# lipku/LiveTalking

Hardware: NVIDIA H100
Metric: lip-sync frames/sec (wav2lip256, 256x256, batch 16, mel + U-Net fwd + paste-back) (higher is better)
Workload: dtype f16 (fp32 accumulate); mel f64; paste u8

## Files before the change

### include/ltb200.h

```cpp
#ifndef LTB200_H_
#define LTB200_H_

#include <stddef.h>
#include <stdint.h>

#ifdef __cplusplus
extern "C" {
#endif

typedef struct ltb_w2l_model ltb_w2l_model;
typedef struct ltb_w2l_avatar ltb_w2l_avatar;
typedef struct ltb_w2l_session ltb_w2l_session;

int ltb_version(void);
const char* ltb_last_error(void);
int ltb_device_count(int* count);
int ltb_set_device(int device);

int ltb_w2l_model_create(const void* blob, size_t nbytes, ltb_w2l_model** out);
int ltb_w2l_model_create_from_device(void* blob_dev, size_t nbytes, ltb_w2l_model** out);
int ltb_w2l_model_destroy(ltb_w2l_model* m);

int ltb_w2l_avatar_create(const uint8_t* faces, const uint8_t* frames, const int32_t* coords, int n, int H, int W,
                          ltb_w2l_avatar** out);
// ... 57 lines not shown
int ltb_ctx_destroy(ltb_ctx* c);
int ltb_ctx_stream(ltb_ctx* c, void** cuda_stream);
int ltb_ctx_sync(ltb_ctx* c);
int ltb_ctx_launch_count(ltb_ctx* c, long long* n);
int ltb_dev_alloc(ltb_ctx* c, size_t bytes, int zero, void** dptr);
int ltb_dev_free(ltb_ctx* c, void* dptr);
int ltb_h2d(ltb_ctx* c, void* dst_dev, const void* src_host, size_t bytes, int sync);
int ltb_d2h(ltb_ctx* c, void* dst_host, const void* src_dev, size_t bytes, int sync);
int ltb_set_i32(ltb_ctx* c, void* dptr, int value);
int ltb_capture_begin(ltb_ctx* c);
int ltb_capture_end(ltb_ctx* c, ltb_graph** out);
int ltb_graph_launch(ltb_ctx* c, ltb_graph* g);
int ltb_graph_destroy(ltb_graph* g);

int ltb_d2d(ltb_ctx* c, void* dst_dev, const void* src_dev, size_t bytes);
typedef struct ltb_conv_op {
  const void* in; const void* w; const void* w_tap; const float* bias; const void* res; void* out;
  int N, IH, IW, ICtot, ic_off, Cin;
  int OH, OW, Cout, OCtot, oc_off, RCtot, rc_off;
  int KH, KW, sy, sx, pad_t, pad_l;
  int Ktot, w_koff, relu, no_halo;
  int zbatch, zdiv;
  long long in_zo, in_zi, w_zo, w_zi, out_zo, out_zi;
  void* gn_stats;
  int gn_groups, gn_hw;
  int upsample2x;
  const int* group_slot;
  int group_images, slots;
  long long w_slot_stride, bias_slot_stride;
  int transposed;
} ltb_conv_op;
int ltb_op_conv2d(ltb_ctx* c, const ltb_conv_op* d);
typedef struct ltb_conv_variant {
  int kernel, taps, bn, nsub, nacc, resident_chunks, kb, ksplit, grouped, res_halo;
} ltb_conv_variant;
int ltb_op_conv2d_plan(ltb_ctx* c, const ltb_conv_op* d, ltb_conv_variant* out);
int ltb_op_w_tap_major(ltb_ctx* c, const void* w, void* wt, int cout, int cin);
int ltb_op_groupnorm(ltb_ctx* c, const void* x, int N, int HW, int C, int Ctot, int c_off, int groups, float eps, const float* gamma,
                     const float* beta, int silu, void* out, int OCtot, int oc_off);
int ltb_op_groupnorm_apply(ltb_ctx* c, const void* x, int N, int HW, int C, int Ctot, int c_off, int groups, float eps, const void* stats,
                           const float* gamma, const float* beta, int silu, void* out, int OCtot, int oc_off);
int ltb_op_layernorm(ltb_ctx* c, const void* x, int rows, int C, float eps, const float* gamma, const float* beta, void* out);
int ltb_op_softmax(ltb_ctx* c, const void* x, int rows, int cols, int ld, int valid, float scale, void* out);
int ltb_op_geglu(ltb_ctx* c, const void* h, long long rows, int H, void* out);
int ltb_op_eltwise(ltb_ctx* c, const void* x, const void* y, long long n, long long period, int act, void* out);
int ltb_op_upsample2x(ltb_ctx* c, const void* x, int N, int H, int W, int C, void* out);
int ltb_op_copy_channels(ltb_ctx* c, const void* src, long long rows, int C, int SCtot, int sc_off, void* dst, int DCtot, int dc_off);
int ltb_op_transpose_heads(ltb_ctx* c, const void* v, int B, int n_keys, int Ctot, int c_off, int heads, int d, int n_pad, void* vt);
int ltb_op_attention(ltb_ctx* c, const void* q, int q_pitch, const void* k, int kv_pitch, int kv_rows, const void* vt, int n_pad, int B, int heads,
                     int nq, int valid, int d, float scale, void* out, int out_pitch);
int ltb_op_dwconv3x3(ltb_ctx* c, const void* x, int N, int IH, int IW, int ICtot, int ic_off, int C, const void* w_tap, const float* bias, int stride,
                     int relu, void* out, int OCtot, int oc_off);
int ltb_op_dwconv3x3_grouped(ltb_ctx* c, const void* x, int N, int IH, int IW, int ICtot, int ic_off, int C, const void* w_tap, const float* bias,
                             int stride, int relu, void* out, int OCtot, int oc_off, const int* group_slot, int group_images, long long w_slot_stride,
                             long long bias_slot_stride);
int ltb_op_upsample_bilinear2x(ltb_ctx* c, const void* x, int N, int H, int W, int ICtot, int ic_off, int C, void* out, int OCtot, int oc_off);
int ltb_op_ul_prep(ltb_ctx* c, const void* faces_u8, int nf, const void* d_index, int B, void* out);
typedef struct ltb_ul_prep_group {
  const void* faces;
  int nf, index;
} ltb_ul_prep_group;
int ltb_op_ul_prep_grouped(ltb_ctx* c, const void* groups_dev, int group_images, int B, void* out);
int ltb_op_head_sigmoid255(ltb_ctx* c, const void* x, const float* w3x32, const float* b3, long long npix, float* pred);
int ltb_op_head_sigmoid255_grouped(ltb_ctx* c, const void* x, const float* w3x32, const float* b3, long long npix, float* pred, int hw,
                                   const int* group_slot, int group_images, long long w_slot_stride, long long bias_slot_stride);
int ltb_op_ul_paste(ltb_ctx* c, const void* frames, const void* faces, const void* coords, const float* pred, void* out, int nf, int H, int W,
                    int index, int explicit_idx, int slot0, int count);
// ... 38 lines not shown
```

### livetalking_b200/_capi.py

```python
from __future__ import annotations

import ctypes as C
import os

_HERE = os.path.dirname(os.path.abspath(__file__))
LIB_PATH = os.path.join(_HERE, "lib", "libltb200.so")

LTB_SESSION_KEEP_LAYERS = 1
LTB_SESSION_NO_GRAPH = 2
LTB_SESSION_NO_HALO = 4
LTB_SESSION_NO_PDL = 8
LTB_SESSION_SLOTS = 16
LTB_SESSION_MEL_ONLY = 32


class LtbError(RuntimeError):
    pass


class ConvOp(C.Structure):
    _fields_ = ([(n, C.c_void_p) for n in ("in_", "w", "w_tap", "bias", "res", "out")] +
                [(n, C.c_int) for n in ("N", "IH", "IW", "ICtot", "ic_off", "Cin", "OH", "OW", "Cout", "OCtot", "oc_off", "RCtot",
                                        "rc_off", "KH", "KW", "sy", "sx", "pad_t", "pad_l", "Ktot", "w_koff", "relu", "no_halo",
                                        "zbatch", "zdiv")] +
                [(n, C.c_longlong) for n in ("in_zo", "in_zi", "w_zo", "w_zi", "out_zo", "out_zi")] +
                [("gn_stats", C.c_void_p), ("gn_groups", C.c_int), ("gn_hw", C.c_int), ("upsample2x", C.c_int)] +
                [("group_slot", C.c_void_p), ("group_images", C.c_int), ("slots", C.c_int), ("w_slot_stride", C.c_longlong),
                 ("bias_slot_stride", C.c_longlong), ("transposed", C.c_int)])


class ConvVariant(C.Structure):
    _fields_ = [(n, C.c_int) for n in ("kernel", "taps", "bn", "nsub", "nacc", "resident_chunks", "kb", "ksplit", "grouped", "res_halo")]


class UlPrepGroup(C.Structure):
    _fields_ = [("faces", C.c_void_p), ("nf", C.c_int), ("index", C.c_int)]


class MtPasteOp(C.Structure):
    _fields_ = ([(n, C.c_void_p) for n in ("frames", "coords", "crop", "masks", "mask_off", "pred", "out")] +
                [(n, C.c_int) for n in ("nf", "H", "W", "index", "explicit_idx", "slot0", "count", "pred_hw")])


class W2LSlot(C.Structure):
    _fields_ = [("avatar", C.c_void_p), ("idx", C.c_int), ("mel", C.c_void_p)]


class ConvDesc(C.Structure):
    _fields_ = [(n, C.c_int) for n in
                ("N", "IH", "IW", "Cin", "Cout", "KH", "KW", "sy", "sx", "pad", "transposed", "relu", "has_res",
                 "force_path")]


_SIGS = {
    "ltb_version": (C.c_int, []),
    "ltb_last_error": (C.c_char_p, []),
    "ltb_device_count": (C.c_int, [C.POINTER(C.c_int)]),
    "ltb_set_device": (C.c_int, [C.c_int]),
    "ltb_w2l_model_create": (C.c_int, [C.c_void_p, C.c_size_t, C.POINTER(C.c_void_p)]),
    "ltb_w2l_model_create_from_device": (C.c_int, [C.c_void_p, C.c_size_t, C.POINTER(C.c_void_p)]),
    "ltb_w2l_model_destroy": (C.c_int, [C.c_void_p]),
    "ltb_w2l_avatar_create": (C.c_int, [C.c_void_p, C.c_void_p, C.c_void_p, C.c_int, C.c_int, C.c_int,
                                        C.POINTER(C.c_void_p)]),
    "ltb_w2l_avatar_destroy": (C.c_int, [C.c_void_p]),
    "ltb_w2l_session_create": (C.c_int, [C.c_void_p, C.c_void_p, C.c_int, C.c_int, C.c_int, C.c_int, C.c_int,
# ... 128 lines not shown
```

### livetalking_b200/csrc/conv_gather.cu

```cuda
#include "conv_params.h"
#include "ltb_internal.h"
#include "ptx_sm90.cuh"

namespace ltb {

constexpr int kGatherThreads = 256;

template <int BN, int KB>
struct GatherCfg {
  static constexpr int CH = KB / 8;
  static constexpr int ROWB = KB * 2;
  static constexpr int RSTEP = kGatherThreads / CH;
  static constexpr int RPT = 128 / RSTEP;
  static constexpr int A_BYTES = 128 * ROWB;
  static constexpr int B_BYTES = (BN * ROWB < 1024) ? 1024 : BN * ROWB;
  static constexpr int STAGE_BYTES = A_BYTES + B_BYTES;
  static constexpr int STAGES = (STAGE_BYTES >= 32768) ? 3 : 4;
  static constexpr uint32_t LAYOUT = (KB == 64) ? 1u : (KB == 32) ? 2u : 3u;
  static constexpr uint32_t SBO = 8 * ROWB;
  static constexpr int SMEM_BYTES = STAGES * STAGE_BYTES + 1024;
};

template <int KB>
__device__ __forceinline__ uint32_t swz_chunk(int row, int j) {
  if (KB == 64) return (uint32_t)(j ^ (row & 7));
  if (KB == 32) return (uint32_t)(j ^ ((row >> 1) & 3));
  return (uint32_t)(j ^ ((row >> 2) & 1));
}

template <int BN, int KB, bool GRP>
__global__ void __launch_bounds__(kGatherThreads) conv_gather_wgmma_kernel(const __grid_constant__ ConvParams p) {
  using C = GatherCfg<BN, KB>;
  extern __shared__ uint8_t smem_raw[];
  const int tid = threadIdx.x;
  const int wg = tid >> 7, wq = (tid >> 5) & 3, lane = tid & 31;
  const uint32_t tiles = (smem_u32(smem_raw) + 1023u) & ~1023u;

  const int zphase = (p.ksplit > 1) ? 0 : ((p.zbatch > 1) ? (int)(blockIdx.z % p.nphases) : (int)blockIdx.z);
  const ConvPhase& ph = p.ph[zphase];
  const __half* in_base = p.in;
  const __half* w_base = p.w;
  __half* out_base = p.out;
  if (p.zbatch > 1) {
    const int zb = blockIdx.z / p.nphases;
    const int zo = zb / p.zdiv, zi = zb - zo * p.zdiv;
    in_base += zo * p.in_zo + zi * p.in_zi;
    w_base += zo * p.w_zo + zi * p.w_zi;
    out_base += zo * p.out_zo + zi * p.out_zi;
  }
  const int g_rows = GRP ? p.group_images * p.GH * p.GW : 0, g_tiles = (g_rows + 127) / 128;
  const int group = GRP ? (int)blockIdx.x / g_tiles : 0;
  const int m0 = GRP ? group * g_rows + ((int)blockIdx.x - group * g_tiles) * 128 : blockIdx.x * 128;
  const int n0 = blockIdx.y * BN;
  const int cpt = p.Cin / KB;
  int it_begin = 0, kiters = ph.ntaps * cpt;
  if (p.ksplit > 1) {
    const int per = (kiters + p.ksplit - 1) / p.ksplit;
    it_begin = (int)blockIdx.z * per;
    kiters = min(per, kiters - it_begin);
  }
  pdl_launch_dependents();
  pdl_wait();
  const float* bias_g = nullptr;
  if constexpr (GRP) {
    const int slot = p.group_slot[group];
    w_base += slot * p.w_slot_stride;
    bias_g = p.bias + slot * p.bias_slot_stride;
  }
  const float* const bias = GRP ? bias_g : p.bias;
  const int M = GRP ? (group + 1) * g_rows : p.M;

  const int j = tid % C::CH;
  const int r0 = tid / C::CH;
  int riy[C::RPT], rix[C::RPT];
  long long rbase[C::RPT];
  const int gsz = p.GH * p.GW;
#pragma unroll
  for (int i = 0; i < C::RPT; ++i) {
    const int m = m0 + r0 + i * C::RSTEP;
    if (m < M) {
      const int b = m / gsz;
      const int rem = m - b * gsz;
      const int gy = rem / p.GW;
      const int gx = rem - gy * p.GW;
      riy[i] = gy * p.sy;
      rix[i] = gx * p.sx;
      rbase[i] = ((long long)(b * p.IH + riy[i]) * p.IW + rix[i]) * p.ICtot + p.ic_off + j * 8;
    } else {
      riy[i] = -(1 << 20);
      rix[i] = 0;
      rbase[i] = 0;
    }
// ... 19 lines not shown
      const int n = r0 + i * C::RSTEP;
      if (n < BN) cp_async16(b_base + n * C::ROWB + swz_chunk<KB>(n, j) * 16, w_base + (size_t)(n0 + n) * p.Ktot + wk, 16u);
    }
  };

  float acc[BN / 2];
#pragma unroll
  for (int i = 0; i < BN / 2; ++i) acc[i] = 0.f;
#pragma unroll
  for (int s = 0; s < C::STAGES - 1; ++s) {
    if (s < kiters) load(s);
    cp_async_commit();
  }
  for (int it = 0; it < kiters; ++it) {
    cp_async_wait<C::STAGES - 2>();
    fence_proxy_async_smem();
    __syncthreads();
    if (it + C::STAGES - 1 < kiters) load(it + C::STAGES - 1);
    cp_async_commit();
    const uint32_t a_base = tiles + (it % C::STAGES) * C::STAGE_BYTES;
    const uint32_t b_base = a_base + C::A_BYTES;
    wgmma_fence();
#pragma unroll
    for (int k = 0; k < KB / 16; ++k) {
      const uint64_t ad = wgmma_desc(a_base + wg * 64 * C::ROWB + k * 32, 16, C::SBO, C::LAYOUT);
      const uint64_t bd = wgmma_desc(b_base + k * 32, 16, C::SBO, C::LAYOUT);
      Wgmma<BN>::ss(acc, ad, bd, 1u);
    }
    wgmma_commit();
    wgmma_wait<0>();
    wgmma_fence_regs(acc);
  }
  cp_async_wait<0>();

  const int cq = 2 * (lane & 3);
#pragma unroll
  for (int hh = 0; hh < 2; ++hh) {
    const int m = m0 + wg * 64 + wq * 16 + (lane >> 2) + 8 * hh;
    if (m >= M) continue;
    if (p.ksplit > 1) {
      float* wrow = p.ws + ((size_t)blockIdx.z * p.M + m) * p.Cout + n0;
#pragma unroll
      for (int i = 0; i < BN / 8; ++i)
        *reinterpret_cast<float2*>(wrow + 8 * i + cq) = make_float2(acc[4 * i + 2 * hh], acc[4 * i + 2 * hh + 1]);
      continue;
    }
    const int b = m / gsz;
    const int rem = m - b * gsz;
    const int gy = rem / p.GW;
    const int gx = rem - gy * p.GW;
    const size_t opix = (size_t)(b * p.OH + gy * p.osy + ph.ooy) * p.OW + gx * p.osx + ph.oox;
    __half* optr = out_base + opix * p.OCtot + p.oc_off + n0;
    const __half* rptr = p.res ? (p.res + opix * p.RCtot + p.rc_off + n0) : nullptr;
#pragma unroll
    for (int i = 0; i < BN / 8; ++i) {
      const int c = 8 * i + cq;
      const float2 bb = __ldg(reinterpret_cast<const float2*>(bias + n0 + c));
      float x = acc[4 * i + 2 * hh] + bb.x, y = acc[4 * i + 2 * hh + 1] + bb.y;
      if (rptr) {
        const float2 rf = __half22float2(__ldcg(reinterpret_cast<const __half2*>(rptr + c)));
        x += rf.x;
        y += rf.y;
      }
      if (p.relu) {
        x = fmaxf(x, 0.f);
        y = fmaxf(y, 0.f);
      }
      x = fminf(fmaxf(x, -65504.f), 65504.f);
      y = fminf(fmaxf(y, -65504.f), 65504.f);
      *reinterpret_cast<__half2*>(optr + c) = __floats2half2_rn(x, y);
    }
  }
}

template <int BN, int KB, bool GRP>
static cudaError_t launch_grp(const ConvParams& p, cudaStream_t st) {
  using C = GatherCfg<BN, KB>;
  static SmemConfigOnce once;
  if (cudaError_t e = once.ensure(conv_gather_wgmma_kernel<BN, KB, GRP>, C::SMEM_BYTES); e != cudaSuccess) return e;
  const int mt = GRP ? (p.N / p.group_images) * ((p.group_images * p.GH * p.GW + 127) / 128) : (p.M + 127) / 128;
  dim3 grid(mt, p.Cout / BN, p.ksplit > 1 ? p.ksplit : p.nphases * (p.zbatch > 1 ? p.zbatch : 1));
  return launch_kernel_pdl(conv_gather_wgmma_kernel<BN, KB, GRP>, grid, dim3(kGatherThreads), C::SMEM_BYTES, st, p);
}

template <int BN, int KB>
static cudaError_t launch_one(const ConvParams& p, cudaStream_t st) {
  return p.group_slot ? launch_grp<BN, KB, true>(p, st) : launch_grp<BN, KB, false>(p, st);
}

template <int KB>
static cudaError_t launch_kb(const ConvParams& p, int bn, cudaStream_t st) {
  switch (bn) {
    case 128: return launch_one<128, KB>(p, st);
    case 64: return launch_one<64, KB>(p, st);
    case 32: return launch_one<32, KB>(p, st);
    case 16: return launch_one<16, KB>(p, st);
  }
  return cudaErrorInvalidValue;
}

static int conv_gather_pick_bn(const ConvParams& p) {
  int bn = 0;
  for (int c : {128, 64, 32, 16})
    if (p.Cout % c == 0) {
      bn = c;
      break;
    }
  if (!bn) return 0;
  const long mt = (p.M + 127) / 128;
  const long zb = p.zbatch > 1 ? p.zbatch : 1;
  while (bn > 32 && mt * (p.Cout / bn) * p.nphases * zb < 132) bn >>= 1;
  return bn;
}
// ... 5 lines not shown
  const unsigned total = (unsigned)M * vpr;
  const size_t slice = (size_t)M * Cout;
  pdl_launch_dependents();
  pdl_wait();
  for (unsigned i = blockIdx.x * 256u + threadIdx.x; i < total; i += gridDim.x * 256u) {
    const size_t m = i / vpr;
    const int c = (int)(i % vpr) * 8;
    float f[8];
#pragma unroll
    for (int j = 0; j < 8; ++j) f[j] = __ldg(bias + c + j);
    for (int s = 0; s < ksplit; ++s) {
      const float4* w4 = reinterpret_cast<const float4*>(ws + s * slice + m * Cout + c);
      const float4 a = __ldcg(w4), b = __ldcg(w4 + 1);
      f[0] += a.x; f[1] += a.y; f[2] += a.z; f[3] += a.w;
      f[4] += b.x; f[5] += b.y; f[6] += b.z; f[7] += b.w;
    }
    if (res) {
      const uint4 rv = __ldcg(reinterpret_cast<const uint4*>(res + m * RCtot + rc_off + c));
      const __half* rh = reinterpret_cast<const __half*>(&rv);
#pragma unroll
      for (int j = 0; j < 8; ++j) f[j] += __half2float(rh[j]);
    }
    uint4 ov;
    __half* oh = reinterpret_cast<__half*>(&ov);
#pragma unroll
    for (int j = 0; j < 8; ++j) {
      float x = relu ? fmaxf(f[j], 0.f) : f[j];
      oh[j] = __float2half_rn(fminf(fmaxf(x, -65504.f), 65504.f));
    }
    *reinterpret_cast<uint4*>(out + m * OCtot + oc_off + c) = ov;
  }
}

bool conv_gather_pick(const ConvParams& p, bool have_ws, size_t splitk_ws_floats, int* bn_out, int* kb_out, int* ksplit_out) {
  if (p.Cout % 16 != 0 || p.Cin % 16 != 0 || (p.ICtot % 8) || (p.OCtot % 8) || (p.ic_off % 8) || (p.oc_off % 8) ||
      (p.Ktot % 8) || p.nphases < 1 || p.nphases > kMaxPhases)
    return false;
  if (p.res && ((p.RCtot % 8) || (p.rc_off % 8))) return false;
  int bn = conv_gather_pick_bn(p);
  if (!bn) return false;
  const int kb = (p.Cin % 64 == 0) ? 64 : (p.Cin % 32 == 0) ? 32 : 16;
  int ksplit = 0;
  const int kiters = p.ph[0].ntaps * (p.Cin / kb);
  const long mt = (p.M + 127) / 128;
  if (have_ws && !p.group_slot && p.nphases == 1 && p.zbatch <= 1 && p.osy == 1 && p.osx == 1 && p.GH == p.OH && p.GW == p.OW && kiters >= 32 && mt <= 8) {
    int bn2 = 0;
    for (int c : {128, 64, 32, 16})
      if (p.Cout % c == 0) {
        bn2 = c;
        break;
      }
    const long tiles = mt * (p.Cout / bn2);
    if (tiles < 64) {
      int ks = (int)((264 + tiles - 1) / tiles);
      if (ks > kiters / 8) ks = kiters / 8;
      if (ks > 32) ks = 32;
      while (ks >= 2 && (size_t)ks * p.M * p.Cout > splitk_ws_floats) --ks;
      if (ks >= 2) {
        const int per = (kiters + ks - 1) / ks;
        ksplit = (kiters + per - 1) / per;
        bn = bn2;
      }
    }
  }
  *bn_out = bn;
  *kb_out = kb;
  *ksplit_out = ksplit;
  return true;
}

cudaError_t launch_conv_gather(const ConvParams& p_in, cudaStream_t st, float* splitk_ws, size_t splitk_ws_floats) {
  ConvParams p = p_in;
  int bn, kb;
  if (!conv_gather_pick(p, splitk_ws != nullptr, splitk_ws_floats, &bn, &kb, &p.ksplit)) return cudaErrorInvalidValue;
  p.ws = p.ksplit > 1 ? splitk_ws : nullptr;
  cudaError_t e;
  if (kb == 64) e = launch_kb<64>(p, bn, st);
  else if (kb == 32) e = launch_kb<32>(p, bn, st);
  else e = launch_kb<16>(p, bn, st);
  if (e != cudaSuccess || p.ksplit <= 1) return e;
  const size_t total = (size_t)p.M * (p.Cout / 8);
  int blocks = (int)((total + 255) / 256);
  if (blocks > 592) blocks = 592;
  return launch_kernel_pdl(splitk_finalize_kernel, dim3(blocks), dim3(256), 0, st, (const float*)p.ws, p.ksplit, p.M, p.Cout, p.bias, p.res,
                           p.RCtot, p.rc_off, p.relu, p.out, p.OCtot, p.oc_off);
}

}
```

### livetalking_b200/csrc/conv_params.h

```cpp
#pragma once
#include <cuda_fp16.h>
#include <cstdint>

namespace ltb {

constexpr int kMaxTaps = 16;
constexpr int kMaxPhases = 4;

struct ConvPhase {
  int ntaps;
  int koff;
  int ooy, oox;
  signed char dy[kMaxTaps];
  signed char dx[kMaxTaps];
};

struct ConvParams {
  const __half* in;
  int N, IH, IW, ICtot, ic_off, Cin;
  int sy, sx;
  int GH, GW;
  __half* out;
  int OH, OW, OCtot, oc_off;
  int osy, osx;
  int Cout;
  const __half* res;
  int RCtot, rc_off;
  const __half* w;
  int Ktot;
  const float* bias;
  int relu;
  int M;
  int nphases;
  ConvPhase ph[kMaxPhases];
  int zbatch, zdiv;
  long long in_zo, in_zi, w_zo, w_zi, out_zo, out_zi;
  int ksplit;
  float* ws;
  int upconv;
  const int* group_slot;
  int group_images, slots;
  long long w_slot_stride, bias_slot_stride;
};

}
```

### livetalking_b200/csrc/conv_plan.cu

```cuda
#include <cstring>
#include <string>
#include <vector>

#include "../../include/ltb200.h"
#include "conv_plan.h"
#include "ltb_internal.h"

namespace ltb {

static const int kTd[2][2] = {{0, 0}, {0, 1}};
static const int kTk[2][2] = {{1, 0}, {2, 0}};
static const int kTn[2] = {1, 2};
static const int kUd[2][2] = {{-1, 0}, {0, 1}};

ConvParams conv_params(ConvMode mode, int N, ConvSlice in, int IH, int IW, int Cin, ConvSlice out, int OH, int OW, int Cout,
                       ConvSlice res, const __half* w, int Ktot, int w_koff, const float* bias, bool relu, ConvTaps taps) {
  ConvParams p;
  std::memset(&p, 0, sizeof(p));
  p.in = in.p;
  p.N = N;
  p.IH = IH;
  p.IW = IW;
  p.ICtot = in.Ctot;
  p.ic_off = in.off;
// ... 35 lines not shown
    p.nphases = 4;
    p.upconv = up ? 1 : 0;
    int koff = w_koff;
    for (int a = 0; a < 2; ++a)
      for (int b = 0; b < 2; ++b) {
        ConvPhase& ph = p.ph[a * 2 + b];
        const int na = up ? 2 : kTn[a], nb = up ? 2 : kTn[b];
        ph.ntaps = na * nb;
        ph.koff = koff;
        ph.ooy = a;
        ph.oox = b;
        for (int i = 0; i < na; ++i)
          for (int j = 0; j < nb; ++j) {
            ph.dy[i * nb + j] = (signed char)(up ? kUd[a][i] : kTd[a][i]);
            ph.dx[i * nb + j] = (signed char)(up ? kUd[b][j] : kTd[b][j]);
          }
        koff += ph.ntaps * Cin;
      }
  }
  p.M = N * p.GH * p.GW;
  return p;
}

int conv_plan(const ConvParams& p, const __half* w_tap, ConvPath path, ConvPlan* out) {
  out->p = p;
  out->halo = false;
  if (p.group_slot) {
    if (p.group_images < 1 || p.N % p.group_images || p.slots < 1 || p.w_slot_stride < 0 || p.bias_slot_stride < 0)
      return LTB_FAIL("conv: grouped weights need N divisible by group_images >= 1, slots >= 1 and non-negative slot strides");
    if (p.zbatch > 1 || p.upconv) return LTB_FAIL("conv: grouped weights cannot be combined with zbatch or the fused upsample");
  }
  if (path == ConvPath::Gather) return 0;
  const bool gemm = p.nphases == 1 && p.ph[0].ntaps == 1;
  if (!((w_tap || gemm) && conv_halo_supported(p))) {
    if (path == ConvPath::Auto) return 0;
    return LTB_FAIL("conv: the halo kernel cannot run " + std::to_string(p.N) + "x" + std::to_string(p.IH) + "x" + std::to_string(p.IW) +
                    "x" + std::to_string(p.Cin) + " -> " + std::to_string(p.OH) + "x" + std::to_string(p.OW) + "x" + std::to_string(p.Cout) +
                    (w_tap || gemm ? "" : " without tap-major weights"));
  }
  if (conv_halo_make_plan(p, w_tap, &out->hp) != 0) return LTB_FAIL("conv: halo plan / tensor map creation failed");
  out->halo = true;
  return 0;
}

cudaError_t conv_launch(const ConvPlan& pl, cudaStream_t st, float* splitk_ws, size_t ws_floats) {
  return pl.halo ? launch_conv_halo(pl.hp, st) : launch_conv_gather(pl.p, st, splitk_ws, ws_floats);
}

bool conv_plan_variant(const ConvPlan& pl, bool have_ws, size_t ws_floats, ltb_conv_variant* out) {
  std::memset(out, 0, sizeof(*out));
  out->grouped = pl.p.group_slot != nullptr;
  if (pl.halo) {
    out->kernel = 1;
    out->taps = pl.hp.TAPS;
    out->bn = pl.hp.BN;
    out->nsub = pl.hp.NSUB;
    out->nacc = pl.hp.NACC;
    out->resident_chunks = conv_halo_resident_chunks(pl.hp, conv_halo_sms());
    out->res_halo = pl.hp.hp.res_halo;
    return true;
  }
  int ksplit = 0;
  if (!conv_gather_pick(pl.p, have_ws, ws_floats, &out->bn, &out->kb, &ksplit)) return false;
  out->ksplit = ksplit > 1 ? ksplit : 1;
  return true;
}

bool conv_plan_fuse_gn_stats(ConvPlan* pl, float* stats, int groups, int hw) {
  const ConvParams& p = pl->p;
  if (!pl->halo || pl->hp.grouped || p.oc_off != 0 || p.OCtot != p.Cout || !conv_halo_gn_fusable(pl->hp, p.Cout, groups, hw)) return false;
  HaloParams& h = pl->hp.hp;
  h.gn_stats = stats;
  h.gn_groups = groups;
  h.gn_cpg = p.Cout / groups;
  h.gn_hw = hw;
  h.gn_images = p.M / hw;
  return true;
}

bool conv_plan_fuse_head(ConvPlan* pl, const float* w, const float* b, float* out) {
  if (!pl->halo || pl->hp.grouped || pl->hp.BN != 32 || pl->p.Cout != 32) return false;
  pl->hp.hp.head_w = w;
  pl->hp.hp.head_b = b;
  pl->hp.hp.head_out = out;
  return true;
}

static void pack_conv_w(const float* w, int cout, int cin, int KH, int KW, std::vector<__half>& out) {
  out.resize((size_t)cout * KH * KW * cin);
  for (int co = 0; co < cout; ++co)
    for (int kh = 0; kh < KH; ++kh)
      for (int kw = 0; kw < KW; ++kw)
        for (int ci = 0; ci < cin; ++ci)
          out[((size_t)co * KH * KW + kh * KW + kw) * cin + ci] = __float2half(w[(((size_t)co * cin + ci) * KH + kh) * KW + kw]);
}
static void pack_convT_w(const float* w, int cin, int cout, std::vector<__half>& out) {
// ... 128 lines not shown
```

### livetalking_b200/csrc/ltb_internal.h

```cpp
#pragma once
#include <cuda_runtime.h>
#include <cuda_fp16.h>
#include <cstdint>
#include <cstdio>
#include <atomic>
#include <cstdlib>
#include <utility>
#include <string>

#include "conv_params.h"

namespace ltb {

void set_error(const std::string& msg);
int fail(const char* file, int line, const std::string& msg);
#define LTB_FAIL(msg) ::ltb::fail(__FILE__, __LINE__, (msg))
#define LTB_CUDA(expr)                                                                         \
  do {                                                                                         \
    cudaError_t _e = (expr);                                                                   \
    if (_e != cudaSuccess) {                                                                   \
      cudaGetLastError();  \
      return LTB_FAIL(std::string(#expr) + ": " + cudaGetErrorString(_e));                     \
    }                                                                                          \
  } while (0)

struct SmemConfigOnce {
  std::atomic<unsigned long long> done{0};
  template <typename K>
  cudaError_t ensure(K kernel, int bytes) {
    int dev = 0;
    cudaError_t e = cudaGetDevice(&dev);
    if (e != cudaSuccess) return e;
    const unsigned long long bit = 1ull << (dev & 63);
    if (done.load(std::memory_order_acquire) & bit) return cudaSuccess;
    e = cudaFuncSetAttribute(kernel, cudaFuncAttributeMaxDynamicSharedMemorySize, bytes);
    if (e == cudaSuccess) done.fetch_or(bit, std::memory_order_release);
    return e;
  }
};

bool pdl_default();
bool pdl_enabled();
void pdl_set_enabled(bool on);

template <typename... KArgs, typename... Args>
inline cudaError_t launch_kernel_pdl(void (*kernel)(KArgs...), dim3 grid, dim3 block, size_t smem, cudaStream_t st, Args&&... args) {
  cudaLaunchConfig_t cfg = {};
  cfg.gridDim = grid;
  cfg.blockDim = block;
  cfg.dynamicSmemBytes = smem;
  cfg.stream = st;
  cudaLaunchAttribute attr[1];
  attr[0].id = cudaLaunchAttributeProgrammaticStreamSerialization;
  attr[0].val.programmaticStreamSerializationAllowed = 1;
  cfg.attrs = attr;
  cfg.numAttrs = pdl_enabled() ? 1 : 0;
  return cudaLaunchKernelEx(&cfg, kernel, std::forward<Args>(args)...);
}

template <typename... KArgs, typename... Args>
inline cudaError_t launch_kernel_plain(void (*kernel)(KArgs...), dim3 grid, dim3 block, size_t smem, cudaStream_t st, Args&&... args) {
  cudaLaunchConfig_t cfg = {};
  cfg.gridDim = grid;
  cfg.blockDim = block;
  cfg.dynamicSmemBytes = smem;
  cfg.stream = st;
  cfg.numAttrs = 0;
  return cudaLaunchKernelEx(&cfg, kernel, std::forward<Args>(args)...);
}

struct SlotDesc {
  const uint8_t* face;
  const uint8_t* frame;
  int y1, y2, x1, x2;
};

cudaError_t launch_conv_gather(const ConvParams& p, cudaStream_t st, float* splitk_ws = nullptr, size_t splitk_ws_floats = 0);
bool conv_gather_pick(const ConvParams& p, bool have_ws, size_t splitk_ws_floats, int* bn, int* kb, int* ksplit);

cudaError_t launch_w2l_prep_faces(const uint8_t* faces, int nfaces, const int* d_index, int B, __half* img_pad, cudaStream_t st,
                                  const SlotDesc* slots = nullptr);
cudaError_t launch_set_int(int* p, int v, cudaStream_t st);
cudaError_t launch_w2l_audio_conv0(const float* mel, const float* w9x32, const float* bias, __half* out, int B, cudaStream_t st);
cudaError_t launch_w2l_head(const __half* x, const float* w3x32, const float* b3, float* pred, int npix, cudaStream_t st);

cudaError_t launch_mel_step(const float* pcm, int nsamp, int B, int stride_left_chunks, int fps, double* scratch_spec,
                            double* scratch_mel, float* out, cudaStream_t st);
size_t mel_scratch_spec_doubles(int nsamp);
size_t mel_scratch_mel_doubles(int nsamp);

cudaError_t launch_w2l_paste(const uint8_t* frames, const int* coords, int nf, int H, int W, const float* pred, int slot0,
                             int index, int explicit_idx, int count, uint8_t* out, cudaStream_t st, const SlotDesc* slots = nullptr);

}
```

### livetalking_b200/csrc/ptx_sm90.cuh

```cuda
#pragma once
#include <cuda_fp16.h>
#include <cstdint>
#include <cstdio>

namespace ltb {

__device__ __forceinline__ uint32_t smem_u32(const void* p) {
  return static_cast<uint32_t>(__cvta_generic_to_shared(p));
}

__device__ __forceinline__ void mbar_init(uint32_t bar, uint32_t count) {
  asm volatile("mbarrier.init.shared::cta.b64 [%0], %1;" ::"r"(bar), "r"(count) : "memory");
}
__device__ __forceinline__ void mbar_fence_init() {
  asm volatile("fence.mbarrier_init.release.cluster;" ::: "memory");
}
__device__ __forceinline__ void mbar_arrive(uint32_t bar) {
  asm volatile("mbarrier.arrive.shared::cta.b64 _, [%0];" ::"r"(bar) : "memory");
}
__device__ __forceinline__ void mbar_arrive_expect_tx(uint32_t bar, uint32_t bytes) {
  asm volatile("mbarrier.arrive.expect_tx.shared::cta.b64 _, [%0], %1;" ::"r"(bar), "r"(bytes) : "memory");
}
__device__ __forceinline__ bool mbar_try_wait(uint32_t bar, uint32_t parity) {
  uint32_t ok;
// ... 232 lines not shown
  }
#undef LTB_R
};

template <>
struct Wgmma<256> {
#define LTB_R "{%0,%1,%2,%3,%4,%5,%6,%7,%8,%9,%10,%11,%12,%13,%14,%15,%16,%17,%18,%19,%20,%21,%22,%23,%24,%25,%26,%27,%28,%29,%30,%31,%32,%33,%34,%35,%36,%37,%38,%39,%40,%41,%42,%43,%44,%45,%46,%47,%48,%49,%50,%51,%52,%53,%54,%55,%56,%57,%58,%59,%60,%61,%62,%63,%64,%65,%66,%67,%68,%69,%70,%71,%72,%73,%74,%75,%76,%77,%78,%79,%80,%81,%82,%83,%84,%85,%86,%87,%88,%89,%90,%91,%92,%93,%94,%95,%96,%97,%98,%99,%100,%101,%102,%103,%104,%105,%106,%107,%108,%109,%110,%111,%112,%113,%114,%115,%116,%117,%118,%119,%120,%121,%122,%123,%124,%125,%126,%127}"
  __device__ __forceinline__ static void ss(float (&d)[128], uint64_t a, uint64_t b, uint32_t acc) {
    asm volatile(LTB_WG_SS("256", LTB_R, "128", "129", "130") : LTB_D128(0) : "l"(a), "l"(b), "r"(acc));
  }
#undef LTB_R
};

template <int N, int C0, int R>
__device__ __forceinline__ void wgmma_ss_at(float (&d)[R], uint64_t a, uint64_t b, uint32_t acc) {
  static_assert(C0 % 8 == 0 && C0 / 2 + N / 2 <= R, "accumulator slice out of range");
  Wgmma<N>::ss(*reinterpret_cast<float(*)[N / 2]>(&d[C0 / 2]), a, b, acc);
}

__device__ __forceinline__ uint32_t f32x2_to_f16x2_sat(float lo, float hi) {
  uint32_t r;
  asm("cvt.rn.satfinite.f16x2.f32 %0, %1, %2;" : "=r"(r) : "f"(hi), "f"(lo));
  return r;
}
__device__ __forceinline__ uint32_t f32x2_to_f16x2_sat_relu(float lo, float hi) {
  uint32_t r;
  asm("cvt.rn.relu.satfinite.f16x2.f32 %0, %1, %2;" : "=r"(r) : "f"(hi), "f"(lo));
  return r;
}

__device__ __forceinline__ void pdl_wait() { asm volatile("griddepcontrol.wait;" ::: "memory"); }
__device__ __forceinline__ void pdl_launch_dependents() { asm volatile("griddepcontrol.launch_dependents;" ::: "memory"); }

template <uint32_t N>
__device__ __forceinline__ void setmaxnreg_inc() {
  asm volatile("setmaxnreg.inc.sync.aligned.u32 %0;" ::"n"(N));
}
template <uint32_t N>
__device__ __forceinline__ void setmaxnreg_dec() {
  asm volatile("setmaxnreg.dec.sync.aligned.u32 %0;" ::"n"(N));
}

__device__ __forceinline__ bool elect_one() {
  uint32_t pred;
  asm volatile(
      "{\n\t.reg .pred p;\n\t"
      "elect.sync _|p, 0xffffffff;\n\t"
      "selp.u32 %0, 1, 0, p;\n\t}"
      : "=r"(pred));
  return pred != 0;
}

}
```

### livetalking_b200/ops.py

```python
from __future__ import annotations

import contextlib
import ctypes as C
from typing import Optional, Sequence

import numpy as np

from . import _capi
from ._capi import ConvOp, MtPasteOp, UlPrepGroup, check, lib


class DevTensor:
    __slots__ = ("ptr", "shape", "dtype", "nbytes", "pitch", "c_off", "stats")

    def __init__(self, ptr: int, shape: Sequence[int], dtype=np.float16, pitch: Optional[int] = None, c_off: int = 0):
        self.ptr = int(ptr)
        self.shape = tuple(int(s) for s in shape)
        self.dtype = np.dtype(dtype)
        self.nbytes = int(np.prod(self.shape)) * self.dtype.itemsize
        self.pitch = int(pitch) if pitch is not None else self.shape[-1]
        self.c_off = int(c_off)
        self.stats = None

    @property
# ... 83 lines not shown
    @property
    def cuda_stream(self) -> int:
        p = C.c_void_p()
        check(lib().ltb_ctx_stream(self._h, C.byref(p)))
        return p.value or 0

    @property
    def launch_count(self) -> int:
        n = C.c_longlong(0)
        check(lib().ltb_ctx_launch_count(self._h, C.byref(n)))
        return n.value

    @contextlib.contextmanager
    def capture(self):
        holder = type("Capture", (), {"graph": None})()
        check(lib().ltb_capture_begin(self._h))
        try:
            yield holder
        except Exception:
            h = C.c_void_p()
            lib().ltb_capture_end(self._h, C.byref(h))
            if h:
                lib().ltb_graph_destroy(h)
            raise
        h = C.c_void_p()
        check(lib().ltb_capture_end(self._h, C.byref(h)))
        holder.graph = Graph(self, h)

    def conv(self, x: DevTensor, w: "ConvWeight", out: DevTensor, **kw):
        check(lib().ltb_op_conv2d(self._h, C.byref(self._conv_op(x, w, out, **kw))))

    def conv_plan(self, x: DevTensor, w: "ConvWeight", out: DevTensor, **kw) -> dict:
        v = self._conv_variant(x, w, out, **kw)
        return {n: getattr(v, n) for n, _ in v._fields_ if n != "res_halo"}

    def conv_res_halo(self, x: DevTensor, w: "ConvWeight", out: DevTensor, **kw) -> bool:
        return bool(self._conv_variant(x, w, out, **kw).res_halo)

    def _conv_variant(self, x: DevTensor, w: "ConvWeight", out: DevTensor, **kw) -> "_capi.ConvVariant":
        v = _capi.ConvVariant()
        check(lib().ltb_op_conv2d_plan(self._h, C.byref(self._conv_op(x, w, out, **kw)), C.byref(v)))
        return v

    def _conv_op(self, x: DevTensor, w: "ConvWeight", out: DevTensor, *, N: int, IH: int, IW: int, OH: int, OW: int, stride=(1, 1),
                 pad=(0, 0), res: Optional[DevTensor] = None, relu: bool = False, cin: Optional[int] = None, no_halo: bool = False,
                 zbatch: int = 0, zdiv: int = 1, in_z=(0, 0), w_z=(0, 0), out_z=(0, 0), w_ptr: Optional[int] = None,
                 ktot: Optional[int] = None, cout: Optional[int] = None, in_ptr: Optional[int] = None, out_ptr: Optional[int] = None,
                 gn_stats: Optional[DevTensor] = None, gn_groups: int = 0, gn_hw: int = 0, upsample2x: bool = False,
                 bias_ptr: Optional[int] = None, group: Optional[tuple] = None, transposed: bool = False) -> ConvOp:
        d = ConvOp()
        d.in_ = in_ptr if in_ptr is not None else x.ptr
        d.w = w_ptr if w_ptr is not None else w.w.ptr
        d.w_tap = (w.w_tap.ptr if (w is not None and w.w_tap is not None and w_ptr is None) else None)
        d.bias = bias_ptr if bias_ptr is not None else (w.bias.ptr if (w is not None and w.bias is not None) else None)
        d.res = res.ptr if res is not None else None
        d.out = out_ptr if out_ptr is not None else out.ptr
        d.N, d.IH, d.IW = N, IH, IW
        d.ICtot, d.ic_off = x.pitch, x.c_off
        d.Cin = cin if cin is not None else w.cin
        d.OH, d.OW = OH, OW
        d.Cout = cout if cout is not None else w.cout
        d.OCtot, d.oc_off = out.pitch, out.c_off
        d.RCtot, d.rc_off = (res.pitch, res.c_off) if res is not None else (0, 0)
        d.KH, d.KW = (w.kh, w.kw) if w is not None else (1, 1)
        d.sy, d.sx = stride
        d.pad_t, d.pad_l = pad
        d.Ktot = ktot if ktot is not None else w.ktot
        d.w_koff = 0
        d.relu = int(relu)
        d.no_halo = int(no_halo)
# ... 241 lines not shown
```

Before: 6926.

## Add cluster-based split-K with DSMEM reduction for small-spatial gather convolutions

Adds a split-K mode for the gather WGMMA conv kernel in which the K-splits run as a thread-block cluster. Partial accumulators are reduced through distributed shared memory, and bias, residual and ReLU are fused into the epilogue, so no global workspace or separate reduce kernel is needed. The split now also covers multi-phase (transposed/strided) convs and picks narrower BN tiles to fill the SMs. The planner routes small-spatial, wide-Cin non-GEMM convs to the gather path instead of the halo kernel. The costs are larger shared memory per block, cluster scheduling constraints, and extra cluster barriers.

```diff
diff --git a/include/ltb200.h b/include/ltb200.h
--- a/include/ltb200.h
+++ b/include/ltb200.h
@@ -113,7 +113,7 @@
 } ltb_conv_op;
 int ltb_op_conv2d(ltb_ctx* c, const ltb_conv_op* d);
 typedef struct ltb_conv_variant {
-  int kernel, taps, bn, nsub, nacc, resident_chunks, kb, ksplit, grouped, res_halo;
+  int kernel, taps, bn, nsub, nacc, resident_chunks, kb, ksplit, grouped, res_halo, cluster;
 } ltb_conv_variant;
 int ltb_op_conv2d_plan(ltb_ctx* c, const ltb_conv_op* d, ltb_conv_variant* out);
 int ltb_op_w_tap_major(ltb_ctx* c, const void* w, void* wt, int cout, int cin);
diff --git a/livetalking_b200/_capi.py b/livetalking_b200/_capi.py
--- a/livetalking_b200/_capi.py
+++ b/livetalking_b200/_capi.py
@@ -30,7 +30,7 @@
 
 
 class ConvVariant(C.Structure):
-    _fields_ = [(n, C.c_int) for n in ("kernel", "taps", "bn", "nsub", "nacc", "resident_chunks", "kb", "ksplit", "grouped", "res_halo")]
+    _fields_ = [(n, C.c_int) for n in ("kernel", "taps", "bn", "nsub", "nacc", "resident_chunks", "kb", "ksplit", "grouped", "res_halo", "cluster")]
 
 
 class UlPrepGroup(C.Structure):
diff --git a/livetalking_b200/csrc/conv_gather.cu b/livetalking_b200/csrc/conv_gather.cu
--- a/livetalking_b200/csrc/conv_gather.cu
+++ b/livetalking_b200/csrc/conv_gather.cu
@@ -19,7 +19,12 @@
   static constexpr uint32_t LAYOUT = (KB == 64) ? 1u : (KB == 32) ? 2u : 3u;
   static constexpr uint32_t SBO = 8 * ROWB;
   static constexpr int SMEM_BYTES = STAGES * STAGE_BYTES + 1024;
+  static constexpr int RED_PITCH = BN + 8;
+  static constexpr int RED_BYTES = 128 * RED_PITCH * 4;
+  static constexpr int CLUSTER_SMEM_BYTES = (RED_BYTES + 1024 > SMEM_BYTES) ? RED_BYTES + 1024 : SMEM_BYTES;
 };
+
+constexpr int kMaxClusterSplit = 8;
 
 template <int KB>
 __device__ __forceinline__ uint32_t swz_chunk(int row, int j) {
@@ -36,7 +41,12 @@
   const int wg = tid >> 7, wq = (tid >> 5) & 3, lane = tid & 31;
   const uint32_t tiles = (smem_u32(smem_raw) + 1023u) & ~1023u;
 
-  const int zphase = (p.ksplit > 1) ? 0 : ((p.zbatch > 1) ? (int)(blockIdx.z % p.nphases) : (int)blockIdx.z);
+  const bool csplit = p.ksplit > 1 && p.cluster;
+  int zphase = (p.zbatch > 1) ? (int)(blockIdx.z % p.nphases) : (int)blockIdx.z, split = 0;
+  if (p.ksplit > 1) {
+    zphase = csplit ? (int)blockIdx.z / p.ksplit : 0;
+    split = (int)blockIdx.z - zphase * p.ksplit;
+  }
   const ConvPhase& ph = p.ph[zphase];
   const __half* in_base = p.in;
   const __half* w_base = p.w;
@@ -56,8 +66,8 @@
   int it_begin = 0, kiters = ph.ntaps * cpt;
   if (p.ksplit > 1) {
     const int per = (kiters + p.ksplit - 1) / p.ksplit;
-    it_begin = (int)blockIdx.z * per;
-    kiters = min(per, kiters - it_begin);
+    it_begin = split * per;
+    kiters = max(0, min(per, kiters - it_begin));
   }
   pdl_launch_dependents();
   pdl_wait();
@@ -143,8 +153,62 @@
     wgmma_fence_regs(acc);
   }
   cp_async_wait<0>();
-
   const int cq = 2 * (lane & 3);
+
+  if (csplit) {
+    __syncthreads();
+    float* red = reinterpret_cast<float*>(smem_raw + (tiles - smem_u32(smem_raw)));
+#pragma unroll
+    for (int hh = 0; hh < 2; ++hh) {
+      float* rrow = red + (wg * 64 + wq * 16 + (lane >> 2) + 8 * hh) * C::RED_PITCH;
+#pragma unroll
+      for (int i = 0; i < BN / 8; ++i)
+        *reinterpret_cast<float2*>(rrow + 8 * i + cq) = make_float2(acc[4 * i + 2 * hh], acc[4 * i + 2 * hh + 1]);
+    }
+    cluster_sync();
+    const int ks = p.ksplit, rows = (128 + ks - 1) / ks;
+    const int r_lo = split * rows, r_hi = min(128, r_lo + rows);
+    constexpr int VPR = BN / 8;
+    for (int v = r_lo * VPR + tid; v < r_hi * VPR; v += kGatherThreads) {
+      const int row = v / VPR, c = (v - row * VPR) * 8;
+      const int m = m0 + row;
+      if (m >= M) continue;
+      const uint32_t la = tiles + (uint32_t)(row * C::RED_PITCH + c) * 4u;
+      float f[8];
+#pragma unroll
+      for (int j = 0; j < 8; ++j) f[j] = 0.f;
+      for (int s = 0; s < ks; ++s) {
+        const uint32_t ra = mapa_shared(la, (uint32_t)s);
+        const float4 a = ld_shared_cluster_f4(ra), b = ld_shared_cluster_f4(ra + 16u);
+        f[0] += a.x; f[1] += a.y; f[2] += a.z; f[3] += a.w;
+        f[4] += b.x; f[5] += b.y; f[6] += b.z; f[7] += b.w;
+      }
+      const int b = m / gsz;
+      const int rem = m - b * gsz;
+      const int gy = rem / p.GW;
+      const int gx = rem - gy * p.GW;
+      const size_t opix = (size_t)(b * p.OH + gy * p.osy + ph.ooy) * p.OW + gx * p.osx + ph.oox;
+#pragma unroll
+      for (int j = 0; j < 8; ++j) f[j] += __ldg(bias + n0 + c + j);
+      if (p.res) {
+        const uint4 rv = __ldcg(reinterpret_cast<const uint4*>(p.res + opix * p.RCtot + p.rc_off + n0 + c));
+        const __half* rh = reinterpret_cast<const __half*>(&rv);
+#pragma unroll
+        for (int j = 0; j < 8; ++j) f[j] += __half2float(rh[j]);
+      }
+      uint4 ov;
+      __half* oh = reinterpret_cast<__half*>(&ov);
+#pragma unroll
+      for (int j = 0; j < 8; ++j) {
+        const float x = p.relu ? fmaxf(f[j], 0.f) : f[j];
+        oh[j] = __float2half_rn(fminf(fmaxf(x, -65504.f), 65504.f));
+      }
+      *reinterpret_cast<uint4*>(out_base + opix * p.OCtot + p.oc_off + n0 + c) = ov;
+    }
+    cluster_sync();
+    return;
+  }
+
 #pragma unroll
   for (int hh = 0; hh < 2; ++hh) {
     const int m = m0 + wg * 64 + wq * 16 + (lane >> 2) + 8 * hh;
@@ -188,8 +252,11 @@
 static cudaError_t launch_grp(const ConvParams& p, cudaStream_t st) {
   using C = GatherCfg<BN, KB>;
   static SmemConfigOnce once;
-  if (cudaError_t e = once.ensure(conv_gather_wgmma_kernel<BN, KB, GRP>, C::SMEM_BYTES); e != cudaSuccess) return e;
+  if (cudaError_t e = once.ensure(conv_gather_wgmma_kernel<BN, KB, GRP>, C::CLUSTER_SMEM_BYTES); e != cudaSuccess) return e;
   const int mt = GRP ? (p.N / p.group_images) * ((p.group_images * p.GH * p.GW + 127) / 128) : (p.M + 127) / 128;
+  if (p.ksplit > 1 && p.cluster)
+    return launch_kernel_pdl_cluster(conv_gather_wgmma_kernel<BN, KB, GRP>, dim3(mt, p.Cout / BN, p.nphases * p.ksplit), dim3(kGatherThreads),
+                                     C::CLUSTER_SMEM_BYTES, st, dim3(1, 1, p.ksplit), p);
   dim3 grid(mt, p.Cout / BN, p.ksplit > 1 ? p.ksplit : p.nphases * (p.zbatch > 1 ? p.zbatch : 1));
   return launch_kernel_pdl(conv_gather_wgmma_kernel<BN, KB, GRP>, grid, dim3(kGatherThreads), C::SMEM_BYTES, st, p);
 }
@@ -261,7 +328,8 @@
   }
 }
 
-bool conv_gather_pick(const ConvParams& p, bool have_ws, size_t splitk_ws_floats, int* bn_out, int* kb_out, int* ksplit_out) {
+bool conv_gather_pick(const ConvParams& p, bool have_ws, size_t splitk_ws_floats, int* bn_out, int* kb_out, int* ksplit_out,
+                      int* cluster_out) {
   if (p.Cout % 16 != 0 || p.Cin % 16 != 0 || (p.ICtot % 8) || (p.OCtot % 8) || (p.ic_off % 8) || (p.oc_off % 8) ||
       (p.Ktot % 8) || p.nphases < 1 || p.nphases > kMaxPhases)
     return false;
@@ -269,45 +337,62 @@
   int bn = conv_gather_pick_bn(p);
   if (!bn) return false;
   const int kb = (p.Cin % 64 == 0) ? 64 : (p.Cin % 32 == 0) ? 32 : 16;
-  int ksplit = 0;
-  const int kiters = p.ph[0].ntaps * (p.Cin / kb);
+  int ksplit = 0, cluster = 0;
+  int kiters = 0;
+  for (int i = 0; i < p.nphases; ++i) kiters = max(kiters, p.ph[i].ntaps * (p.Cin / kb));
   const long mt = (p.M + 127) / 128;
-  if (have_ws && !p.group_slot && p.nphases == 1 && p.zbatch <= 1 && p.osy == 1 && p.osx == 1 && p.GH == p.OH && p.GW == p.OW && kiters >= 32 && mt <= 8) {
+  if (!p.group_slot && p.zbatch <= 1 && kiters >= 32 && mt <= 8) {
     int bn2 = 0;
     for (int c : {128, 64, 32, 16})
       if (p.Cout % c == 0) {
         bn2 = c;
         break;
       }
-    const long tiles = mt * (p.Cout / bn2);
-    if (tiles < 64) {
-      int ks = (int)((264 + tiles - 1) / tiles);
-      if (ks > kiters / 8) ks = kiters / 8;
-      if (ks > 32) ks = 32;
-      while (ks >= 2 && (size_t)ks * p.M * p.Cout > splitk_ws_floats) --ks;
-      if (ks >= 2) {
-        const int per = (kiters + ks - 1) / ks;
-        ksplit = (kiters + per - 1) / per;
-        bn = bn2;
-      }
+    long tiles = mt * (p.Cout / bn2) * p.nphases;
+    int ks = 0;
+    if (have_ws && p.nphases == 1 && p.osy == 1 && p.osx == 1 && p.GH == p.OH && p.GW == p.OW) {
+      if (tiles < 64) {
+        ks = (int)((264 + tiles - 1) / tiles);
+        if (ks > kiters / 8) ks = kiters / 8;
+        if (ks > 32) ks = 32;
+        while (ks >= 2 && (size_t)ks * p.M * p.Cout > splitk_ws_floats) --ks;
+      }
+    } else if (kiters <= kMaxClusterSplit * 16 && reinterpret_cast<uintptr_t>(p.out) % 16 == 0 &&
+               (!p.res || reinterpret_cast<uintptr_t>(p.res) % 16 == 0)) {
+      ks = min(kMaxClusterSplit, kiters / 16);
+      if (ks > 132 / tiles) ks = (int)(132 / tiles);
+      if (ks == kMaxClusterSplit)
+        while (bn2 > 32 && 2 * tiles * ks <= 132) {
+          bn2 >>= 1;
+          tiles <<= 1;
+        }
+      cluster = 1;
+    }
+    if (ks >= 2) {
+      const int per = (kiters + ks - 1) / ks;
+      ksplit = (kiters + per - 1) / per;
+      bn = bn2;
+    } else {
+      cluster = 0;
     }
   }
   *bn_out = bn;
   *kb_out = kb;
   *ksplit_out = ksplit;
+  *cluster_out = cluster;
   return true;
 }
 
 cudaError_t launch_conv_gather(const ConvParams& p_in, cudaStream_t st, float* splitk_ws, size_t splitk_ws_floats) {
   ConvParams p = p_in;
   int bn, kb;
-  if (!conv_gather_pick(p, splitk_ws != nullptr, splitk_ws_floats, &bn, &kb, &p.ksplit)) return cudaErrorInvalidValue;
-  p.ws = p.ksplit > 1 ? splitk_ws : nullptr;
+  if (!conv_gather_pick(p, splitk_ws != nullptr, splitk_ws_floats, &bn, &kb, &p.ksplit, &p.cluster)) return cudaErrorInvalidValue;
+  p.ws = (p.ksplit > 1 && !p.cluster) ? splitk_ws : nullptr;
   cudaError_t e;
   if (kb == 64) e = launch_kb<64>(p, bn, st);
   else if (kb == 32) e = launch_kb<32>(p, bn, st);
   else e = launch_kb<16>(p, bn, st);
-  if (e != cudaSuccess || p.ksplit <= 1) return e;
+  if (e != cudaSuccess || p.ksplit <= 1 || p.cluster) return e;
   const size_t total = (size_t)p.M * (p.Cout / 8);
   int blocks = (int)((total + 255) / 256);
   if (blocks > 592) blocks = 592;
diff --git a/livetalking_b200/csrc/conv_params.h b/livetalking_b200/csrc/conv_params.h
--- a/livetalking_b200/csrc/conv_params.h
+++ b/livetalking_b200/csrc/conv_params.h
@@ -35,7 +35,7 @@
   ConvPhase ph[kMaxPhases];
   int zbatch, zdiv;
   long long in_zo, in_zi, w_zo, w_zi, out_zo, out_zi;
-  int ksplit;
+  int ksplit, cluster;
   float* ws;
   int upconv;
   const int* group_slot;
diff --git a/livetalking_b200/csrc/conv_plan.cu b/livetalking_b200/csrc/conv_plan.cu
--- a/livetalking_b200/csrc/conv_plan.cu
+++ b/livetalking_b200/csrc/conv_plan.cu
@@ -91,6 +91,7 @@
   }
   if (path == ConvPath::Gather) return 0;
   const bool gemm = p.nphases == 1 && p.ph[0].ntaps == 1;
+  if (path == ConvPath::Auto && !gemm && !p.upconv && p.GH * p.GW <= 16 && p.Cin >= 8 * 64) return 0;
   if (!((w_tap || gemm) && conv_halo_supported(p))) {
     if (path == ConvPath::Auto) return 0;
     return LTB_FAIL("conv: the halo kernel cannot run " + std::to_string(p.N) + "x" + std::to_string(p.IH) + "x" + std::to_string(p.IW) +
@@ -120,7 +121,7 @@
     return true;
   }
   int ksplit = 0;
-  if (!conv_gather_pick(pl.p, have_ws, ws_floats, &out->bn, &out->kb, &ksplit)) return false;
+  if (!conv_gather_pick(pl.p, have_ws, ws_floats, &out->bn, &out->kb, &ksplit, &out->cluster)) return false;
   out->ksplit = ksplit > 1 ? ksplit : 1;
   return true;
 }
diff --git a/livetalking_b200/csrc/ltb_internal.h b/livetalking_b200/csrc/ltb_internal.h
--- a/livetalking_b200/csrc/ltb_internal.h
+++ b/livetalking_b200/csrc/ltb_internal.h
@@ -44,18 +44,32 @@
 void pdl_set_enabled(bool on);
 
 template <typename... KArgs, typename... Args>
-inline cudaError_t launch_kernel_pdl(void (*kernel)(KArgs...), dim3 grid, dim3 block, size_t smem, cudaStream_t st, Args&&... args) {
+inline cudaError_t launch_kernel_pdl_cluster(void (*kernel)(KArgs...), dim3 grid, dim3 block, size_t smem, cudaStream_t st, dim3 cluster,
+                                             Args&&... args) {
   cudaLaunchConfig_t cfg = {};
   cfg.gridDim = grid;
   cfg.blockDim = block;
   cfg.dynamicSmemBytes = smem;
   cfg.stream = st;
-  cudaLaunchAttribute attr[1];
-  attr[0].id = cudaLaunchAttributeProgrammaticStreamSerialization;
-  attr[0].val.programmaticStreamSerializationAllowed = 1;
+  cudaLaunchAttribute attr[2];
+  unsigned n = 0;
+  if (pdl_enabled()) {
+    attr[n].id = cudaLaunchAttributeProgrammaticStreamSerialization;
+    attr[n++].val.programmaticStreamSerializationAllowed = 1;
+  }
+  if (cluster.x * cluster.y * cluster.z > 1) {
+    attr[n].id = cudaLaunchAttributeClusterDimension;
+    attr[n].val.clusterDim.x = cluster.x;
+    attr[n].val.clusterDim.y = cluster.y;
+    attr[n++].val.clusterDim.z = cluster.z;
+  }
   cfg.attrs = attr;
-  cfg.numAttrs = pdl_enabled() ? 1 : 0;
+  cfg.numAttrs = n;
   return cudaLaunchKernelEx(&cfg, kernel, std::forward<Args>(args)...);
+}
+template <typename... KArgs, typename... Args>
+inline cudaError_t launch_kernel_pdl(void (*kernel)(KArgs...), dim3 grid, dim3 block, size_t smem, cudaStream_t st, Args&&... args) {
+  return launch_kernel_pdl_cluster(kernel, grid, block, smem, st, dim3(1, 1, 1), std::forward<Args>(args)...);
 }
 
 template <typename... KArgs, typename... Args>
@@ -76,7 +90,7 @@
 };
 
 cudaError_t launch_conv_gather(const ConvParams& p, cudaStream_t st, float* splitk_ws = nullptr, size_t splitk_ws_floats = 0);
-bool conv_gather_pick(const ConvParams& p, bool have_ws, size_t splitk_ws_floats, int* bn, int* kb, int* ksplit);
+bool conv_gather_pick(const ConvParams& p, bool have_ws, size_t splitk_ws_floats, int* bn, int* kb, int* ksplit, int* cluster);
 
 cudaError_t launch_w2l_prep_faces(const uint8_t* faces, int nfaces, const int* d_index, int B, __half* img_pad, cudaStream_t st,
                                   const SlotDesc* slots = nullptr);
diff --git a/livetalking_b200/csrc/ptx_sm90.cuh b/livetalking_b200/csrc/ptx_sm90.cuh
--- a/livetalking_b200/csrc/ptx_sm90.cuh
+++ b/livetalking_b200/csrc/ptx_sm90.cuh
@@ -288,6 +288,20 @@
 __device__ __forceinline__ void pdl_wait() { asm volatile("griddepcontrol.wait;" ::: "memory"); }
 __device__ __forceinline__ void pdl_launch_dependents() { asm volatile("griddepcontrol.launch_dependents;" ::: "memory"); }
 
+__device__ __forceinline__ void cluster_sync() {
+  asm volatile("barrier.cluster.arrive.release.aligned;\n\tbarrier.cluster.wait.acquire.aligned;" ::: "memory");
+}
+__device__ __forceinline__ uint32_t mapa_shared(uint32_t addr, uint32_t rank) {
+  uint32_t r;
+  asm volatile("mapa.shared::cluster.u32 %0, %1, %2;" : "=r"(r) : "r"(addr), "r"(rank));
+  return r;
+}
+__device__ __forceinline__ float4 ld_shared_cluster_f4(uint32_t addr) {
+  float4 v;
+  asm volatile("ld.shared::cluster.v4.f32 {%0, %1, %2, %3}, [%4];" : "=f"(v.x), "=f"(v.y), "=f"(v.z), "=f"(v.w) : "r"(addr) : "memory");
+  return v;
+}
+
 template <uint32_t N>
 __device__ __forceinline__ void setmaxnreg_inc() {
   asm volatile("setmaxnreg.inc.sync.aligned.u32 %0;" ::"n"(N));
diff --git a/livetalking_b200/ops.py b/livetalking_b200/ops.py
--- a/livetalking_b200/ops.py
+++ b/livetalking_b200/ops.py
@@ -139,10 +139,14 @@
 
     def conv_plan(self, x: DevTensor, w: "ConvWeight", out: DevTensor, **kw) -> dict:
         v = self._conv_variant(x, w, out, **kw)
-        return {n: getattr(v, n) for n, _ in v._fields_ if n != "res_halo"}
+        return {n: getattr(v, n) for n, _ in v._fields_ if n not in ("res_halo", "cluster")}
 
     def conv_res_halo(self, x: DevTensor, w: "ConvWeight", out: DevTensor, **kw) -> bool:
         return bool(self._conv_variant(x, w, out, **kw).res_halo)
+
+    def conv_cluster_split(self, x: DevTensor, w: "ConvWeight", out: DevTensor, **kw) -> int:
+        v = self._conv_variant(x, w, out, **kw)
+        return v.ksplit if v.cluster else 0
 
     def _conv_variant(self, x: DevTensor, w: "ConvWeight", out: DevTensor, **kw) -> "_capi.ConvVariant":
         v = _capi.ConvVariant()
```

Result: no change. 6904 (median of 6 runs) (-0.3%).
